# godk1122/IsaacLab

Measured on AMD Instinct MI355X. Metric: env-steps/sec (whole node), Anymal-C rough 4096 envs/GPU, RSL-RL PPO iteration (collect+GAE+update), higher is better.
Workload: dtype f32; 1 GPU; Isaac-Velocity-Rough-Anymal-C-v0, 4096 envs/GPU, T=24, 5 epochs x 4 minibatches, terrain 1204008 triangles, 4 state snapshots resident in HBM; parallelism=dp1, rollout=hipGraph, full_step=False, update=hipGraph (measured eager 16.90 ms, graph 16.30 ms), policy_params=571801

## Files before the change

isaaclab_amd/csrc/mlp.hip:

```cpp
#include <algorithm>

#include "imx_internal.h"

typedef float f32x16 __attribute__((ext_vector_type(16)));

namespace {

constexpr int DW_T = 128;
constexpr int DW_BM = 32;
constexpr int DW_LD = DW_T + 32;

struct DwArgs {
    int64_t M;
    int N, K;
    const float* dY;
    int64_t ldy;
    const float* X;
    int64_t ldx;
    float* part;
    float* part_db;
    int tn, tk, S;
    int64_t rps;
    const float* H;
    int64_t ldh;
// ... 283 lines not shown
    const int64_t i = (int64_t)(blockIdx.x - g.first_block) * 64 + tx;
    const float* src = nullptr;
    int64_t stride = 0;
    float* dst = nullptr;
    if (i < g.total) {
        src = g.part + i; stride = g.total; dst = g.out + i;
    } else if (g.db && i - g.total < g.N) {
        src = g.part_db + (i - g.total); stride = g.N; dst = g.db + (i - g.total);
    }
    float acc = 0.0f;
    if (src)
        for (int s = ty; s < g.S; s += RED_Y) acc += src[(size_t)s * stride];
    red[ty][tx] = acc;
    __syncthreads();
    if (ty == 0 && dst) {
        float sum = 0.0f;
#pragma unroll
        for (int y = 0; y < RED_Y; ++y) sum += red[y][tx];
        *dst = sum;
    }
}

struct DwPlan {
    int tn, tk, S;
    int64_t rps;
};

int g_num_cu = 0;
int g_dw_cu_budget = 0;

DwPlan dw_plan(int64_t M, int N, int K) {
    if (g_num_cu == 0) {
        int dev = 0, cu = 0;
        if (hipGetDevice(&dev) != hipSuccess || hipDeviceGetAttribute(&cu, hipDeviceAttributeMultiprocessorCount, dev) != hipSuccess || cu <= 0)
            cu = 256;
        g_num_cu = cu;
    }
    DwPlan p;
    p.tn = (N + DW_T - 1) / DW_T;
    p.tk = (K + DW_T - 1) / DW_T;
    const int T = p.tn * p.tk;
    const int cus = g_dw_cu_budget > 0 ? std::min(g_dw_cu_budget, g_num_cu) : g_num_cu;
    int64_t S = std::max<int64_t>(1, (int64_t)cus / T);
    S = std::min<int64_t>(S, std::max<int64_t>(1, M / (2 * DW_BM)));
    if (S >= 8) S &= ~(int64_t)7;
    p.rps = ((M + S - 1) / S + DW_BM - 1) / DW_BM * DW_BM;
    p.S = (int)((M + p.rps - 1) / p.rps);
    return p;
}

constexpr int HEAD_A = 64;

#define IMX_HALF_LOG_2PI_F 0.91893853320467274178f
template <bool ELU_IN, int AMAX, int LOSS>
__global__ void __launch_bounds__(256) k_head_fwd(int64_t M, int K, int A, float* __restrict__ h, int64_t ldh,
                                                  const float* __restrict__ W, const float* __restrict__ b, float* __restrict__ y,
                                                  float alpha, imx_head_loss_t L) {
    extern __shared__ float sW[];
    for (int i = threadIdx.x; i < A * K; i += blockDim.x) sW[i] = W[i];
    __syncthreads();
    const int q = threadIdx.x & 3;
    const int64_t row = (int64_t)blockIdx.x * 64 + (threadIdx.x >> 2);
    const bool live = row < M;
    float acc[AMAX];
#pragma unroll
    for (int o = 0; o < AMAX; ++o) acc[o] = 0.0f;
    float* hr = h + (live ? row : 0) * ldh;
    for (int k = 4 * q; k < K; k += 16) {
        float4 hv = *reinterpret_cast<const float4*>(hr + k);
        if (ELU_IN) {
            const float ex = (expf(fminf(hv.x, 0.0f)) - 1.0f) * alpha, ey = (expf(fminf(hv.y, 0.0f)) - 1.0f) * alpha;
            const float ez = (expf(fminf(hv.z, 0.0f)) - 1.0f) * alpha, ew = (expf(fminf(hv.w, 0.0f)) - 1.0f) * alpha;
            hv.x = hv.x > 0.0f ? hv.x : ex; hv.y = hv.y > 0.0f ? hv.y : ey; hv.z = hv.z > 0.0f ? hv.z : ez; hv.w = hv.w > 0.0f ? hv.w : ew;
            if (live) *reinterpret_cast<float4*>(hr + k) = hv;
        }
#pragma unroll
        for (int o = 0; o < AMAX; ++o)
            if (o < A) {
                const float4 wv = *reinterpret_cast<const float4*>(sW + o * K + k);
                acc[o] = fmaf(hv.w, wv.w, fmaf(hv.z, wv.z, fmaf(hv.y, wv.y, fmaf(hv.x, wv.x, acc[o]))));
            }
    }
#pragma unroll
    for (int o = 0; o < AMAX; ++o) {
        float v = acc[o];
        v += __shfl_xor(v, 1);
        v += __shfl_xor(v, 2);
        acc[o] = v + b[o < A ? o : 0];
    }
    if (q == 0 && live) {
#pragma unroll
        for (int o = 0; o < AMAX; ++o)
            if (o < A) y[row * A + o] = acc[o];
        if (LOSS == 1) {
            const float inv_m = L.grad_scale / (float)M;
            float logp = 0.0f;
#pragma unroll
            for (int o = 0; o < AMAX; ++o)
                if (o < A) {
                    const float m = acc[o], s = L.sigma_d[row * L.sigma_stride + o];
                    const float d = L.actions_d[row * A + o] - m;
                    logp += -(d * d) / (2.0f * s * s) - logf(s) - IMX_HALF_LOG_2PI_F;
                }
            const float ratio = expf(logp - L.old_logp_d[row]);
            const float ad = L.advantages_d[row], clip = L.clip_param;
            const float s1 = -ad * ratio, s2 = -ad * fminf(fmaxf(ratio, 1.0f - clip), 1.0f + clip);
            float dsur_dlogp;
            if (s1 >= s2) dsur_dlogp = -ad * ratio;
            else dsur_dlogp = (ratio > 1.0f - clip && ratio < 1.0f + clip) ? -ad * ratio : 0.0f;
            const float g = dsur_dlogp * inv_m;
#pragma unroll
            for (int o = 0; o < AMAX; ++o)
                if (o < A) {
                    const float m = acc[o], s = L.sigma_d[row * L.sigma_stride + o];
                    const float d = L.actions_d[row * A + o] - m;
                    L.dmu_d[row * A + o] = g * (d / (s * s));
                    L.dsigma_d[row * A + o] = g * ((d * d) / (s * s * s) - 1.0f / s) - L.entropy_coef * inv_m / s;
                }
        } else if (LOSS == 2) {
            const float inv_m = L.grad_scale / (float)M;
            const float v = acc[0], R = L.returns_d[row], clip = L.clip_param;
            float dv;
            if (L.use_clipped_value_loss) {
                const float vo = L.old_values_d[row];
                const float dlt = v - vo;
                const float vc = vo + fminf(fmaxf(dlt, -clip), clip);
                const float l1 = (v - R) * (v - R), l2 = (vc - R) * (vc - R);
                if (l1 >= l2) dv = 2.0f * (v - R);
                else dv = (dlt > -clip && dlt < clip) ? 2.0f * (vc - R) : 0.0f;
            } else {
                dv = -2.0f * (R - v);
            }
            L.dvalue_d[row] = L.value_loss_coef * dv * inv_m;
        }
    }
}

template <int AB>
__global__ void __launch_bounds__(512) k_head_bwd(int64_t M, int K, int A, const float* __restrict__ dY, const float* __restrict__ h,
                                                    int64_t ldh, const float* __restrict__ W, float alpha, int has_act,
                                                    float* __restrict__ dprev, float* __restrict__ part, float* __restrict__ part_db) {
    const int lane = threadIdx.x & 63, kb = threadIdx.x >> 6, r = lane & 31, half = lane >> 5;
    const int kc = kb * 32 + r;
    const int steps = (A + 1) >> 1;
    float wreg[AB * 16];
#pragma unroll
    for (int s = 0; s < AB * 16; ++s) {
        const int o = 2 * s + half;
        wreg[s] = (s < steps && o < A) ? W[o * K + kc] : 0.0f;
    }
    f32x16 wacc[AB];
    float dbacc[AB];
#pragma unroll
    for (int b = 0; b < AB; ++b) {
        dbacc[b] = 0.0f;
#pragma unroll
        for (int q = 0; q < 16; ++q) wacc[b][q] = 0.0f;
    }
    __shared__ float sdy[2][32 * (HEAD_A + 1)];
    const int P = A | 1;
    const int64_t nblk = (M + 31) / 32;
    int buf = 0;
    for (int64_t rb = blockIdx.x; rb < nblk; rb += gridDim.x, buf ^= 1) {
        const int64_t m0 = rb * 32;
        {
            const int64_t base = m0 * A, lim = M * (int64_t)A;
            for (int e = threadIdx.x; e < 32 * A; e += blockDim.x) {
                const int row = e / A, col = e - row * A;
                sdy[buf][row * P + col] = base + e < lim ? dY[base + e] : 0.0f;
            }
        }
        __syncthreads();
        const float* __restrict__ ty = sdy[buf];
        float hv[16];
#pragma unroll
        for (int q = 0; q < 16; ++q) {
            const int64_t row = m0 + acc_row(q, half);
            hv[q] = row < M ? h[row * ldh + kc] : 0.0f;
        }
        f32x16 dx;
#pragma unroll
        for (int q = 0; q < 16; ++q) dx[q] = 0.0f;
#pragma unroll
        for (int s = 0; s < AB * 16; ++s)
            if (s < steps) {
                const int o = 2 * s + half;
                const float av = o < A ? ty[r * P + o] : 0.0f;
                dx = __builtin_amdgcn_mfma_f32_32x32x2f32(av, wreg[s], dx, 0, 0, 0);
            }
        if (m0 + 32 <= M) {
#pragma unroll
            for (int q = 0; q < 16; ++q) {
                const float g = (has_act && hv[q] <= 0.0f) ? hv[q] + alpha : 1.0f;
                dprev[(m0 + acc_row(q, half)) * (int64_t)K + kc] = dx[q] * g;
            }
        } else {
#pragma unroll
            for (int q = 0; q < 16; ++q) {
                const int64_t row = m0 + acc_row(q, half);
                const float g = (has_act && hv[q] <= 0.0f) ? hv[q] + alpha : 1.0f;
                if (row < M) dprev[row * (int64_t)K + kc] = dx[q] * g;
            }
        }
#pragma unroll
        for (int q = 0; q < 16; ++q) {
#pragma unroll
            for (int b = 0; b < AB; ++b) {
                const int o = 32 * b + r;
                const float av = o < A ? ty[acc_row(q, half) * P + o] : 0.0f;
                wacc[b] = __builtin_amdgcn_mfma_f32_32x32x2f32(av, hv[q], wacc[b], 0, 0, 0);
                dbacc[b] += av;
            }
        }
    }
    float* p = part + (size_t)blockIdx.x * A * K;
#pragma unroll
    for (int b = 0; b < AB; ++b) {
#pragma unroll
        for (int q = 0; q < 16; ++q) {
            const int o = 32 * b + acc_row(q, half);
            if (o < A) p[o * K + kc] = wacc[b][q];
        }
        if (kb == 0) {
            const float tot = dbacc[b] + __shfl_xor(dbacc[b], 32);
            if (half == 0 && 32 * b + r < A) part_db[(size_t)blockIdx.x * A + 32 * b + r] = tot;
        }
    }
}

template <int K, int AMAX, int LOSS, bool ELU_IN>
__global__ void __launch_bounds__(2 * K) k_head_fused(int64_t M, int A, const float* __restrict__ z, int64_t ldz, const float* __restrict__ W,
                                                      const float* __restrict__ bias, float alpha, float* __restrict__ y, imx_head_loss_t L,
                                                      float* __restrict__ dprev, float* __restrict__ part, float* __restrict__ part_db) {
    constexpr int AB = (AMAX + 31) / 32;
    extern __shared__ float smem[];
    constexpr int P = K + 32;
    const int PA = A | 1;
    float* sW = smem;
    float* sh = sW + ((A * K + 3) & ~3);
    float* sdy = sh + 2 * 32 * P;
    float* sbs = sdy + 32 * PA;
    constexpr int T = 2 * K;
    const int lane = threadIdx.x & 63, kb = threadIdx.x >> 6, r = lane & 31, half = lane >> 5;
    const int kc = kb * 32 + r;
    constexpr int tpr = T >> 5;
    const int frow = threadIdx.x / tpr, fpart = threadIdx.x - frow * tpr;
    for (int i = threadIdx.x; i < A * K; i += T) sW[i] = W[i];
    if (threadIdx.x < AMAX) {
        sbs[threadIdx.x] = threadIdx.x < A ? bias[threadIdx.x] : 0.0f;
        if (LOSS == 1) sbs[AMAX + threadIdx.x] = (threadIdx.x < A && L.sigma_stride == 0) ? L.sigma_d[threadIdx.x] : 1.0f;
    }
    const int steps = (A + 1) >> 1;
    float wreg[AB * 16];
#pragma unroll
    for (int s = 0; s < AB * 16; ++s) {
        const int o = 2 * s + half;
        wreg[s] = (s < steps && o < A) ? W[o * K + kc] : 0.0f;
    }
    f32x16 wacc[AB];
    float dbacc[AB];
#pragma unroll
    for (int b = 0; b < AB; ++b) {
        dbacc[b] = 0.0f;
#pragma unroll
        for (int q = 0; q < 16; ++q) wacc[b][q] = 0.0f;
    }
    constexpr int kq = K >> 2;
    const int64_t nblk = (M + 31) / 32;
    float4 zt[4];
    constexpr int JCAP = LOSS == 1 ? (AMAX + tpr - 1) / tpr : 1;
    float la[JCAP], ls[JCAP], l0 = 0.0f, l1 = 0.0f;
    const bool own_sigma = LOSS == 1 && L.sigma_stride != 0;
    auto load_tile = [&](int64_t rb) {
        {
            const int64_t grow = rb * 32 + frow < M ? rb * 32 + frow : M - 1;
            if (LOSS == 1) {
#pragma unroll
                for (int j = 0; j < JCAP; ++j) {
                    const int o = fpart + tpr * j;
                    la[j] = L.actions_d[grow * A + (o < A ? o : 0)];
// ... 301 lines not shown
    IMX_REQUIRE(t_batch == nullptr, "imx_reduce_batch_begin: another batch is still open on this thread (flush it first)");
    t_batch = b;
    return 0;
}

extern "C" int imx_reduce_batch_flush(imx_reduce_batch_t* b, imx_stream_t stream) {
    IMX_REQUIRE(b && t_batch == b, "imx_reduce_batch_flush: this batch is not the one open on this thread");
    t_batch = nullptr;
    if (b->args.n == 0) return 0;
    hipLaunchKernelGGL(k_mlp_reduce_batch, dim3(b->blocks), dim3(64, RED_Y), 0, (hipStream_t)stream, b->args);
    b->args.n = 0;
    b->blocks = 0;
    IMX_HIP(hipGetLastError());
    return 0;
}

extern "C" int imx_mlp_dw(int64_t M, int N, int K, const float* dY_d, int64_t ldy, const float* X_d, int64_t ldx, float* dW_d,
                          float* db_d, void* scratch_d, size_t scratch_bytes, imx_stream_t stream) {
    return mlp_dw_launch("imx_mlp_dw", M, N, K, dY_d, ldy, nullptr, 0, 0.0f, nullptr, 0, X_d, ldx, dW_d, db_d, scratch_d, scratch_bytes,
                         stream);
}

extern "C" int imx_mlp_dw_elu(int64_t M, int N, int K, const float* dH_d, int64_t ldg, const float* H_d, int64_t ldh, float elu_alpha,
                              float* dZ_out_d, int64_t ldd, const float* X_d, int64_t ldx, float* dW_d, float* db_d, void* scratch_d,
                              size_t scratch_bytes, imx_stream_t stream) {
    IMX_REQUIRE(H_d, "imx_mlp_dw_elu: the saved activation output is required");
    return mlp_dw_launch("imx_mlp_dw_elu", M, N, K, dH_d, ldg, H_d, ldh, elu_alpha, dZ_out_d, ldd, X_d, ldx, dW_d, db_d, scratch_d,
                         scratch_bytes, stream);
}

static int head_fwd_launch(int64_t M, int K, int A, float* h_d, int64_t ldh, const float* W_d, const float* b_d, float* y_d,
                           int elu_in_place, float elu_alpha, const imx_head_loss_t* loss, imx_stream_t stream) {
    IMX_REQUIRE(M > 0 && h_d && W_d && b_d && y_d, "imx_mlp_head_fwd: bad arguments");
    IMX_REQUIRE(A >= 1 && A <= HEAD_A, "imx_mlp_head_fwd: %d outputs (1..%d supported; wider layers are library GEMMs)", A, HEAD_A);
    IMX_REQUIRE(K >= 16 && K % 16 == 0 && K <= 2048 && ldh >= K && ldh % 4 == 0 && aligned16(h_d),
                "imx_mlp_head_fwd: in-features %d (pitch %lld) must be a multiple of 16, 16-byte aligned rows", K, (long long)ldh);
    IMX_REQUIRE((size_t)A * K * sizeof(float) <= 64 * 1024, "imx_mlp_head_fwd: %d x %d weights do not fit the 64 KB of LDS used", A, K);
    imx_head_loss_t L{};
    int mode = 0;
    if (loss) {
        L = *loss;
        mode = L.mode;
        IMX_REQUIRE(mode == 1 || mode == 2, "imx_mlp_head_fwd_loss: mode %d (1 policy, 2 value)", mode);
        if (mode == 1) {
            IMX_REQUIRE(L.sigma_d && L.actions_d && L.old_logp_d && L.advantages_d && L.dmu_d && L.dsigma_d, "imx_mlp_head_fwd_loss: null policy argument");
            IMX_REQUIRE(L.sigma_stride == 0 || L.sigma_stride == A, "imx_mlp_head_fwd_loss: sigma_stride must be 0 (shared std) or A");
        } else {
            IMX_REQUIRE(A == 1 && L.returns_d && L.dvalue_d && (!L.use_clipped_value_loss || L.old_values_d), "imx_mlp_head_fwd_loss: value head needs A = 1, returns, old values");
        }
    }
    const dim3 grid((unsigned)((M + 63) / 64)), block(256);
    const size_t lds = (size_t)A * K * sizeof(float);
    hipStream_t st = (hipStream_t)stream;
#define IMX_HEAD_FWD(E, AM, LS) hipLaunchKernelGGL((k_head_fwd<E, AM, LS>), grid, block, lds, st, M, K, A, h_d, ldh, W_d, b_d, y_d, elu_alpha, L)
#define IMX_HEAD_FWD_E(AM, LS) do { if (elu_in_place) IMX_HEAD_FWD(true, AM, LS); else IMX_HEAD_FWD(false, AM, LS); } while (0)
    if (A <= 16) {
        if (mode == 0) IMX_HEAD_FWD_E(16, 0); else if (mode == 1) IMX_HEAD_FWD_E(16, 1); else IMX_HEAD_FWD_E(16, 2);
    } else {
        if (mode == 0) IMX_HEAD_FWD_E(HEAD_A, 0); else if (mode == 1) IMX_HEAD_FWD_E(HEAD_A, 1); else IMX_HEAD_FWD_E(HEAD_A, 2);
    }
#undef IMX_HEAD_FWD_E
#undef IMX_HEAD_FWD
    IMX_HIP(hipGetLastError());
    return 0;
}

extern "C" int imx_mlp_head_fwd(int64_t M, int K, int A, float* h_d, int64_t ldh, const float* W_d, const float* b_d, float* y_d,
                                int elu_in_place, float elu_alpha, imx_stream_t stream) {
    return head_fwd_launch(M, K, A, h_d, ldh, W_d, b_d, y_d, elu_in_place, elu_alpha, nullptr, stream);
}

extern "C" int imx_mlp_head_fwd_loss(int64_t M, int K, int A, float* h_d, int64_t ldh, const float* W_d, const float* b_d, float* y_d,
                                     int elu_in_place, float elu_alpha, const imx_head_loss_t* loss, imx_stream_t stream) {
    IMX_REQUIRE(loss, "imx_mlp_head_fwd_loss: null loss description");
    return head_fwd_launch(M, K, A, h_d, ldh, W_d, b_d, y_d, elu_in_place, elu_alpha, loss, stream);
}

extern "C" int imx_mlp_head_bwd(int64_t M, int K, int A, const float* dY_d, const float* h_d, int64_t ldh, const float* W_d, float elu_alpha,
                                int has_activation, float* dprev_d, float* dW_d, float* db_d, void* scratch_d, size_t scratch_bytes,
                                imx_stream_t stream) {
    IMX_REQUIRE(M > 0 && dY_d && h_d && W_d && dprev_d && dW_d && db_d && scratch_d, "imx_mlp_head_bwd: bad arguments");
    IMX_REQUIRE(A >= 1 && A <= HEAD_A, "imx_mlp_head_bwd: %d outputs (1..%d supported)", A, HEAD_A);
    IMX_REQUIRE(K >= 32 && K % 32 == 0 && K <= 256 && ldh >= K, "imx_mlp_head_bwd: in-features %d must be a multiple of 32, at most 256", K);
    const int G = head_grid(M);
    const size_t need = ((size_t)G * A * K + (size_t)G * A) * sizeof(float);
    IMX_REQUIRE(scratch_bytes >= need, "imx_mlp_head_bwd: scratch too small (%zu < %zu bytes)", scratch_bytes, need);
    float* part = (float*)scratch_d;
    float* part_db = part + (size_t)G * A * K;
    hipStream_t st = (hipStream_t)stream;
    if (A <= 32)
        hipLaunchKernelGGL((k_head_bwd<1>), dim3((unsigned)G), dim3((unsigned)(K / 32 * 64)), 0, st, M, K, A, dY_d, h_d, ldh, W_d, elu_alpha,
                           has_activation, dprev_d, part, part_db);
    else
        hipLaunchKernelGGL((k_head_bwd<2>), dim3((unsigned)G), dim3((unsigned)(K / 32 * 64)), 0, st, M, K, A, dY_d, h_d, ldh, W_d, elu_alpha,
                           has_activation, dprev_d, part, part_db);
    IMX_HIP(hipGetLastError());
    return reduce_or_defer("imx_mlp_head_bwd", (int64_t)A * K, G, part, dW_d, A, part_db, db_d, st);
}

extern "C" int imx_mlp_head_fwd_bwd(int64_t M, int K, int A, const float* z_d, int64_t ldz, const float* W_d, const float* b_d, float* y_d,
                                    int elu_in, float elu_alpha, const imx_head_loss_t* loss, float* dprev_d, float* dW_d, float* db_d,
                                    void* scratch_d, size_t scratch_bytes, imx_reduce_batch_t* defer_to, imx_stream_t stream) {
    IMX_REQUIRE(M > 0 && z_d && W_d && b_d && y_d && loss && dprev_d && dW_d && db_d && scratch_d, "imx_mlp_head_fwd_bwd: bad arguments");
    IMX_REQUIRE(A >= 1 && A <= HEAD_A, "imx_mlp_head_fwd_bwd: %d outputs (1..%d supported)", A, HEAD_A);
    IMX_REQUIRE((K == 128 || K == 256) && ldz >= K && ldz % 4 == 0 && aligned16(z_d),
                "imx_mlp_head_fwd_bwd: in-features %d (pitch %lld) must be 128 or 256 with 16-byte aligned rows", K, (long long)ldz);
    IMX_REQUIRE(A <= 16, "imx_mlp_head_fwd_bwd: %d outputs (at most 16: wider heads run as imx_mlp_head_fwd_loss + imx_mlp_head_bwd)", A);
    const imx_head_loss_t L = *loss;
    IMX_REQUIRE(L.mode == 1 || L.mode == 2, "imx_mlp_head_fwd_bwd: loss mode %d (1 = policy, 2 = value)", L.mode);
    if (L.mode == 1) {
        IMX_REQUIRE(L.sigma_d && L.actions_d && L.old_logp_d && L.advantages_d && L.dmu_d && L.dsigma_d, "imx_mlp_head_fwd_bwd: null policy argument");
        IMX_REQUIRE(L.sigma_stride == 0 || L.sigma_stride == A, "imx_mlp_head_fwd_bwd: sigma_stride must be 0 (shared std) or A");
    } else {
        IMX_REQUIRE(A == 1 && L.returns_d && L.dvalue_d && (!L.use_clipped_value_loss || L.old_values_d),
                    "imx_mlp_head_fwd_bwd: value head needs A = 1, returns, old values");
    }
    const int G = head_grid(M);
    const size_t need = ((size_t)G * A * K + (size_t)G * A) * sizeof(float);
    IMX_REQUIRE(scratch_bytes >= need, "imx_mlp_head_fwd_bwd: scratch too small (%zu < %zu bytes)", scratch_bytes, need);
    float* part = (float*)scratch_d;
    float* part_db = part + (size_t)G * A * K;
    hipStream_t st = (hipStream_t)stream;
    const size_t lds = ((size_t)((A * K + 3) & ~3) + 2ull * 32 * (K + 32) + 32ull * (A | 1) + 2 * HEAD_A) * sizeof(float);
    const dim3 grid((unsigned)G), block((unsigned)(2 * K));
#define IMX_HEAD_FUSED(K_, AM, LS, E)                                                                                                      \
    do {                                                                                                                                  \
        static bool attr = false;                                                                                                         \
        if (!attr) {                                                                                                                      \
            IMX_HIP(hipFuncSetAttribute(reinterpret_cast<const void*>(k_head_fused<K_, AM, LS, E>), hipFuncAttributeMaxDynamicSharedMemorySize, \
                                        160 * 1024));                                                                                    \
            attr = true;                                                                                                                  \
        }                                                                                                                                 \
        hipLaunchKernelGGL((k_head_fused<K_, AM, LS, E>), grid, block, lds, st, M, A, z_d, ldz, W_d, b_d, elu_alpha, y_d, L, dprev_d, part, \
                           part_db);                                                                                                      \
    } while (0)
#define IMX_HEAD_FUSED_K(AM, LS, E) do { if (K == 128) IMX_HEAD_FUSED(128, AM, LS, E); else IMX_HEAD_FUSED(256, AM, LS, E); } while (0)
    if (L.mode == 2) {
        if (elu_in) IMX_HEAD_FUSED_K(1, 2, true); else IMX_HEAD_FUSED_K(1, 2, false);
    } else {
        if (elu_in) IMX_HEAD_FUSED_K(16, 1, true); else IMX_HEAD_FUSED_K(16, 1, false);
    }
#undef IMX_HEAD_FUSED_K
#undef IMX_HEAD_FUSED
    IMX_HIP(hipGetLastError());
    if (defer_to) {
        imx_reduce_batch* saved = t_batch;
        t_batch = defer_to;
        const int rc = reduce_or_defer("imx_mlp_head_fwd_bwd", (int64_t)A * K, G, part, dW_d, A, part_db, db_d, st);
// ... 535 lines not shown
```

isaaclab_amd/csrc/rollout.hip:

```cpp
#include "imx_internal.h"

struct Mom {
    float n, mean, m2;
};
IMX_DEV Mom mom_merge(Mom a, Mom b) {
    Mom r;
    r.n = a.n + b.n;
    if (r.n == 0.0f) { r.mean = 0.0f; r.m2 = 0.0f; return r; }
    const float d = b.mean - a.mean;
    r.mean = a.mean + d * (b.n / r.n);
    r.m2 = a.m2 + b.m2 + d * d * (a.n * b.n / r.n);
    return r;
}
IMX_DEV Mom mom_wave(Mom m) {
#pragma unroll
    for (int o = 32; o > 0; o >>= 1) {
        Mom b;
        b.n = __shfl_xor(m.n, o, 64);
        b.mean = __shfl_xor(m.mean, o, 64);
        b.m2 = __shfl_xor(m.m2, o, 64);
        const bool lo = ((threadIdx.x & o) == 0);
        m = lo ? mom_merge(m, b) : mom_merge(b, m);
    }
    return m;
// ... 126 lines not shown
    for (int u = GAE_TMAX - 1; u >= 0; --u) {
        if (u < T) {
            const float nnt = 1.0f - (d[u] ? 1.0f : 0.0f);
            const float delta = r[u] + nnt * gamma * next_v - v[u];
            advantage = delta + nnt * gamma * lam * advantage;
            const float rt = advantage + v[u];
            const float at = rt - v[u];
            if (live) {
                ret[(int64_t)u * N + e] = rt;
                adv[(int64_t)u * N + e] = at;
            }
            m.n += 1.0f;
            const float dd = at - m.mean;
            m.mean += dd / m.n;
            m.m2 += dd * (at - m.mean);
            next_v = v[u];
        }
    }
    if (!live) m = Mom{0.0f, 0.0f, 0.0f};
    m = mom_wave(m);
    if (threadIdx.x == 0) {
        scratch[3 * blockIdx.x + 0] = m.n;
        scratch[3 * blockIdx.x + 1] = m.mean;
        scratch[3 * blockIdx.x + 2] = m.m2;
    }
}

extern "C" int imx_gae(int64_t T, int64_t N, const float* rew, const float* val, const uint8_t* dones,
                       const float* last_val, float gamma, float lam, int normalize, float* ret, float* adv,
                       void* scratch, imx_stream_t stream) {
    IMX_REQUIRE(T > 0 && N > 0, "imx_gae: empty rollout (T=%lld N=%lld)", (long long)T, (long long)N);
    IMX_REQUIRE(rew && val && dones && last_val && ret && adv && scratch, "imx_gae: null argument");
    const unsigned nblk = (unsigned)((N + GAE_BLOCK - 1) / GAE_BLOCK);
    if (T <= GAE_TMAX)
        hipLaunchKernelGGL(k_gae_short, dim3(nblk), dim3(GAE_BLOCK), 0, (hipStream_t)stream, (int)T, N, rew, val, dones, last_val, gamma, lam,
                           ret, adv, (float*)scratch);
    else
        hipLaunchKernelGGL(k_gae, dim3(nblk), dim3(GAE_BLOCK), 0, (hipStream_t)stream, T, N, rew, val, dones, last_val, gamma, lam,
                           ret, adv, (float*)scratch);
    IMX_HIP(hipGetLastError());
    if (normalize) {
        const int64_t total = T * N;
        const unsigned grid = (unsigned)std::min<int64_t>((total / 4 + 255) / 256 + 1, 1024);
        hipLaunchKernelGGL(k_adv_normalize, dim3(grid), dim3(256), 0, (hipStream_t)stream, total, (int)nblk,
                           (const float*)scratch, adv);
        IMX_HIP(hipGetLastError());
    }
    return 0;
}


extern "C" size_t imx_ppo_scratch_bytes(int64_t M) { return ((size_t)((M + 255) / 256) * 4 + 8) * sizeof(float); }

__global__ void __launch_bounds__(256)
k_ppo_fwd(int64_t M, int A, const float* __restrict__ mu, const float* __restrict__ sigma, int sigma_stride,
          const float* __restrict__ act, const float* __restrict__ old_logp, const float* __restrict__ old_mu,
          const float* __restrict__ old_sigma, const float* __restrict__ adv, const float* __restrict__ ret,
          const float* __restrict__ val, const float* __restrict__ old_val, float clip, int clipped_value,
          float* __restrict__ part) {
    const int64_t i = (int64_t)blockIdx.x * blockDim.x + threadIdx.x;
    float sur = 0.0f, vl = 0.0f, ent = 0.0f, kl = 0.0f;
    if (i < M) {
        float logp = 0.0f;
        for (int a = 0; a < A; ++a) {
            const float m = mu[i * A + a], s = sigma[i * sigma_stride + a];
            const float d = act[i * A + a] - m;
            const float ls = logf(s);
            logp += -(d * d) / (2.0f * s * s) - ls - IMX_HALF_LOG_2PI;
            ent += 0.5f + IMX_HALF_LOG_2PI + ls;
            if (old_mu) {
                const float mo = old_mu[i * A + a], so = old_sigma[i * A + a];
                const float dm = mo - m;
                kl += logf(s / so + 1.0e-5f) + (so * so + dm * dm) / (2.0f * s * s) - 0.5f;
            }
        }
        const float ratio = expf(logp - old_logp[i]);
        const float ad = adv[i];
        const float s1 = -ad * ratio, s2 = -ad * fminf(fmaxf(ratio, 1.0f - clip), 1.0f + clip);
        sur = fmaxf(s1, s2);
        const float v = val[i], R = ret[i];
        if (clipped_value) {
            const float vo = old_val[i];
            const float vc = vo + fminf(fmaxf(v - vo, -clip), clip);
            const float l1 = (v - R) * (v - R), l2 = (vc - R) * (vc - R);
            vl = fmaxf(l1, l2);
        } else {
            vl = (R - v) * (R - v);
        }
    }
    __shared__ float sm[4][4];
    float r4[4] = {sur, vl, ent, kl};
#pragma unroll
    for (int q = 0; q < 4; ++q) {
        float x = r4[q];
#pragma unroll
        for (int o = 32; o > 0; o >>= 1) x += __shfl_xor(x, o, 64);
        if ((threadIdx.x & 63) == 0) sm[threadIdx.x >> 6][q] = x;
    }
    __syncthreads();
    if (threadIdx.x < 4) part[4 * blockIdx.x + threadIdx.x] = (sm[0][threadIdx.x] + sm[1][threadIdx.x]) + (sm[2][threadIdx.x] + sm[3][threadIdx.x]);
}

__global__ void k_ppo_finish(int nblk, float inv_m, float vcoef, float ecoef, const float* __restrict__ part,
                             float* __restrict__ out8, float* __restrict__ accum) {
    __shared__ float red[16][4];
    __shared__ float r[4];
    const int q = threadIdx.x & 3, chunk = threadIdx.x >> 2;
    float s = 0.0f;
    for (int b = chunk; b < nblk; b += 16) s += part[4 * b + q];
    red[chunk][q] = s;
    __syncthreads();
    if (threadIdx.x < 4) {
        float tot = 0.0f;
        for (int c = 0; c < 16; ++c) tot += red[c][threadIdx.x];
        r[threadIdx.x] = tot * inv_m;
        out8[threadIdx.x] = r[threadIdx.x];
    }
    __syncthreads();
    if (threadIdx.x == 0) {
        out8[4] = r[0] + vcoef * r[1] - ecoef * r[2];
        if (accum) {
            accum[0] += r[1]; accum[1] += r[0]; accum[2] += r[2]; accum[3] += r[3]; accum[4] += 1.0f;
        }
    }
}

// ... 4 lines not shown
          int clipped_value, float vcoef, float ecoef, float gscale, float* __restrict__ dmu,
          float* __restrict__ dsigma, float* __restrict__ dval) {
    const int64_t i = (int64_t)blockIdx.x * blockDim.x + threadIdx.x;
    if (i >= M) return;
    const float inv_m = gscale / (float)M;
    if (dmu) {
        float logp = 0.0f;
        for (int a = 0; a < A; ++a) {
            const float m = mu[i * A + a], s = sigma[i * sigma_stride + a];
            const float d = act[i * A + a] - m;
            logp += -(d * d) / (2.0f * s * s) - logf(s) - IMX_HALF_LOG_2PI;
        }
        const float ratio = expf(logp - old_logp[i]);
        const float ad = adv[i];
        const float s1 = -ad * ratio, s2 = -ad * fminf(fmaxf(ratio, 1.0f - clip), 1.0f + clip);
        float dsur_dlogp;
        if (s1 >= s2) dsur_dlogp = -ad * ratio;
        else dsur_dlogp = (ratio > 1.0f - clip && ratio < 1.0f + clip) ? -ad * ratio : 0.0f;
        const float g = dsur_dlogp * inv_m;
        for (int a = 0; a < A; ++a) {
            const float m = mu[i * A + a], s = sigma[i * sigma_stride + a];
            const float d = act[i * A + a] - m;
            dmu[i * A + a] = g * (d / (s * s));
            dsigma[i * A + a] = g * ((d * d) / (s * s * s) - 1.0f / s) - ecoef * inv_m / s;
        }
    }
    if (!dval) return;
    const float v = val[i], R = ret[i];
    float dv;
    if (clipped_value) {
        const float vo = old_val[i];
        const float dlt = v - vo;
        const float vc = vo + fminf(fmaxf(dlt, -clip), clip);
        const float l1 = (v - R) * (v - R), l2 = (vc - R) * (vc - R);
        if (l1 >= l2) dv = 2.0f * (v - R);
        else dv = (dlt > -clip && dlt < clip) ? 2.0f * (vc - R) : 0.0f;
    } else {
        dv = -2.0f * (R - v);
    }
    dval[i] = vcoef * dv * inv_m;
}

extern "C" int imx_ppo_loss_fwd(int64_t M, int64_t A, const float* mu, const float* sigma, int64_t sigma_stride,
                                const float* act, const float* old_logp, const float* old_mu, const float* old_sigma,
                                const float* adv, const float* ret, const float* val, const float* old_val, float clip,
                                int clipped_value, float vcoef, float ecoef, float* out8, float* accum, void* scratch,
                                imx_stream_t stream) {
    IMX_REQUIRE(M > 0 && A > 0 && A <= 4096, "imx_ppo_loss_fwd: bad sizes M=%lld A=%lld", (long long)M, (long long)A);
    IMX_REQUIRE(sigma_stride == 0 || sigma_stride == A, "imx_ppo_loss_fwd: sigma_stride must be 0 (shared std) or A");
    IMX_REQUIRE(mu && sigma && act && old_logp && adv && ret && val && out8 && scratch, "imx_ppo_loss_fwd: null argument");
    IMX_REQUIRE(!clipped_value || old_val, "imx_ppo_loss_fwd: clipped value loss needs old values");
    IMX_REQUIRE((old_mu == nullptr) == (old_sigma == nullptr), "imx_ppo_loss_fwd: old_mu/old_sigma must come together");
    const unsigned nblk = (unsigned)((M + 255) / 256);
    hipLaunchKernelGGL(k_ppo_fwd, dim3(nblk), dim3(256), 0, (hipStream_t)stream, M, (int)A, mu, sigma, (int)sigma_stride, act,
                       old_logp, old_mu, old_sigma, adv, ret, val, old_val, clip, clipped_value, (float*)scratch);
    hipLaunchKernelGGL(k_ppo_finish, dim3(1), dim3(64), 0, (hipStream_t)stream, (int)nblk, 1.0f / (float)M, vcoef, ecoef,
                       (const float*)scratch, out8, accum);
    IMX_HIP(hipGetLastError());
    return 0;
}

extern "C" int imx_ppo_loss_bwd(int64_t M, int64_t A, const float* mu, const float* sigma, int64_t sigma_stride,
                                const float* act, const float* old_logp, const float* adv, const float* ret, const float* val,
                                const float* old_val, float clip, int clipped_value, float vcoef, float ecoef, float gscale,
                                float* dmu, float* dsigma, float* dval, imx_stream_t stream) {
    IMX_REQUIRE(M > 0 && A > 0, "imx_ppo_loss_bwd: bad sizes");
    IMX_REQUIRE(sigma_stride == 0 || sigma_stride == A, "imx_ppo_loss_bwd: sigma_stride must be 0 (shared std) or A");
    IMX_REQUIRE(dmu || dval, "imx_ppo_loss_bwd: nothing to compute (dmu and dval are both null)");
    IMX_REQUIRE(!dmu || (mu && sigma && act && old_logp && adv && dsigma), "imx_ppo_loss_bwd: the policy part needs mu, sigma, "
                "actions, old log-prob, advantages and dsigma");
    IMX_REQUIRE(!dval || (ret && val), "imx_ppo_loss_bwd: the value part needs returns and values");
    IMX_REQUIRE(!dval || !clipped_value || old_val, "imx_ppo_loss_bwd: clipped value loss needs old values");
    hipLaunchKernelGGL(k_ppo_bwd, dim3((unsigned)((M + 255) / 256)), dim3(256), 0, (hipStream_t)stream, M, (int)A, mu, sigma,
                       (int)sigma_stride, act, old_logp, adv, ret, val, old_val, clip, clipped_value, vcoef, ecoef, gscale, dmu,
                       dsigma, dval);
    IMX_HIP(hipGetLastError());
    return 0;
}

__global__ void __launch_bounds__(256)
k_adam(int64_t n, float* __restrict__ p, const float* __restrict__ g, float* __restrict__ m, float* __restrict__ v,
       const float* __restrict__ lr_d, const float* __restrict__ norm_d, float max_norm, float b1, float b2, float eps,
       float bias1, float sqrt_bias2) {
    const float lr = lr_d[0];
    float coef = 1.0f;
    if (norm_d) coef = fminf(max_norm / (norm_d[0] + 1.0e-6f), 1.0f);
    const float step_size = lr / bias1;
    for (int64_t i = (int64_t)blockIdx.x * blockDim.x + threadIdx.x; i < n; i += (int64_t)gridDim.x * blockDim.x) {
        const float gi = g[i] * coef;
        const float mi = b1 * m[i] + (1.0f - b1) * gi;
        const float vi = b2 * v[i] + (1.0f - b2) * gi * gi;
        m[i] = mi;
        v[i] = vi;
        p[i] = p[i] - step_size * (mi / (sqrtf(vi) / sqrt_bias2 + eps));
    }
}

extern "C" int imx_adam_step(int64_t n, float* p, const float* g, float* m, float* v, const float* lr_d,
                             const float* grad_norm_d, float max_norm, float beta1, float beta2, float eps,
                             int64_t step, imx_stream_t stream) {
    IMX_REQUIRE(n > 0 && p && g && m && v && lr_d && step > 0, "imx_adam_step: bad arguments");
    const float bias1 = 1.0f - powf(beta1, (float)step);
    const float sb2 = sqrtf(1.0f - powf(beta2, (float)step));
    const unsigned grid = (unsigned)std::min<int64_t>((n + 255) / 256, 2048);
    hipLaunchKernelGGL(k_adam, dim3(grid), dim3(256), 0, (hipStream_t)stream, n, p, g, m, v, lr_d, grad_norm_d, max_norm,
                       beta1, beta2, eps, bias1, sb2);
    IMX_HIP(hipGetLastError());
    return 0;
// ... 316 lines not shown
```

Baseline: 5.238 million env-steps/s.

## Specialize MLP head kernels for K=128/256 with prefetch and software pipelining

Adds compile-time K specializations to the head forward kernel. Activations and loss inputs are loaded before the weight copy into shared memory, so global latency overlaps the weight staging. Adds a software-pipelined head backward kernel that fetches the next row block of dY and h into registers while MFMA work runs on the current block. Also specializes the PPO loss forward for A=12/37, batching all loads ahead of the math. The cost is more register pressure and more template instances, and the specialized paths only cover the listed sizes.

```diff
diff --git a/isaaclab_amd/csrc/mlp.hip b/isaaclab_amd/csrc/mlp.hip
--- a/isaaclab_amd/csrc/mlp.hip
+++ b/isaaclab_amd/csrc/mlp.hip
@@ -359,13 +359,44 @@
 constexpr int HEAD_A = 64;
 
 #define IMX_HALF_LOG_2PI_F 0.91893853320467274178f
-template <bool ELU_IN, int AMAX, int LOSS>
+__device__ __forceinline__ float4 head_elu4(float4 hv, float alpha) {
+    const float ex = (expf(fminf(hv.x, 0.0f)) - 1.0f) * alpha, ey = (expf(fminf(hv.y, 0.0f)) - 1.0f) * alpha;
+    const float ez = (expf(fminf(hv.z, 0.0f)) - 1.0f) * alpha, ew = (expf(fminf(hv.w, 0.0f)) - 1.0f) * alpha;
+    hv.x = hv.x > 0.0f ? hv.x : ex; hv.y = hv.y > 0.0f ? hv.y : ey; hv.z = hv.z > 0.0f ? hv.z : ez; hv.w = hv.w > 0.0f ? hv.w : ew;
+    return hv;
+}
+
+template <int AMAX>
+__device__ __forceinline__ void head_dot4(float (&acc)[AMAX], float4 hv, const float* sWk, int K, int A) {
+#pragma unroll
+    for (int o = 0; o < AMAX; ++o)
+        if (o < A) {
+            const float4 wv = *reinterpret_cast<const float4*>(sWk + o * K);
+            acc[o] = fmaf(hv.w, wv.w, fmaf(hv.z, wv.z, fmaf(hv.y, wv.y, fmaf(hv.x, wv.x, acc[o]))));
+        }
+}
+
+template <int NMAX>
+__device__ __forceinline__ void head_weights_to_lds(float* sW, const float* __restrict__ W, int n) {
+#pragma unroll
+    for (int c = 0; c < (NMAX + 2047) / 2048; ++c) {
+        const int i0 = c * 2048 + threadIdx.x;
+        if (c * 2048 < n) {
+            float w[8];
+#pragma unroll
+            for (int j = 0; j < 8; ++j) w[j] = W[min(i0 + 256 * j, n - 1)];
+#pragma unroll
+            for (int j = 0; j < 8; ++j)
+                if (i0 + 256 * j < n) sW[i0 + 256 * j] = w[j];
+        }
+    }
+}
+
+template <bool ELU_IN, int AMAX, int LOSS, int KT>
 __global__ void __launch_bounds__(256) k_head_fwd(int64_t M, int K, int A, float* __restrict__ h, int64_t ldh,
                                                   const float* __restrict__ W, const float* __restrict__ b, float* __restrict__ y,
                                                   float alpha, imx_head_loss_t L) {
     extern __shared__ float sW[];
-    for (int i = threadIdx.x; i < A * K; i += blockDim.x) sW[i] = W[i];
-    __syncthreads();
     const int q = threadIdx.x & 3;
     const int64_t row = (int64_t)blockIdx.x * 64 + (threadIdx.x >> 2);
     const bool live = row < M;
@@ -373,20 +404,53 @@
 #pragma unroll
     for (int o = 0; o < AMAX; ++o) acc[o] = 0.0f;
     float* hr = h + (live ? row : 0) * ldh;
-    for (int k = 4 * q; k < K; k += 16) {
-        float4 hv = *reinterpret_cast<const float4*>(hr + k);
+    constexpr bool PRE = LOSS != 0 && AMAX <= 16;
+    float pa[PRE && LOSS == 1 ? AMAX : 1], ps[PRE && LOSS == 1 ? AMAX : 1], p0 = 0.0f, p1 = 0.0f;
+    if constexpr (PRE) {
+        const int64_t rc = live ? row : 0;
+        if (LOSS == 1) {
+#pragma unroll
+            for (int o = 0; o < AMAX; ++o) {
+                pa[o] = L.actions_d[rc * A + (o < A ? o : 0)];
+                ps[o] = L.sigma_d[rc * L.sigma_stride + (o < A ? o : 0)];
+            }
+            p0 = L.old_logp_d[rc];
+            p1 = L.advantages_d[rc];
+        } else {
+            p0 = L.returns_d[rc];
+            p1 = L.use_clipped_value_loss ? L.old_values_d[rc] : 0.0f;
+        }
+    }
+    auto sig = [&](int o) { if constexpr (PRE) return ps[o]; else return L.sigma_d[row * L.sigma_stride + o]; };
+    auto act = [&](int o) { if constexpr (PRE) return pa[o]; else return L.actions_d[row * A + o]; };
+    if constexpr (KT > 0) {
+        constexpr int NT = KT / 16;
+        float4 hv[NT];
+#pragma unroll
+        for (int t = 0; t < NT; ++t) hv[t] = *reinterpret_cast<const float4*>(hr + 4 * q + 16 * t);
+        head_weights_to_lds<AMAX * KT>(sW, W, A * KT);
+        __syncthreads();
         if (ELU_IN) {
-            const float ex = (expf(fminf(hv.x, 0.0f)) - 1.0f) * alpha, ey = (expf(fminf(hv.y, 0.0f)) - 1.0f) * alpha;
-            const float ez = (expf(fminf(hv.z, 0.0f)) - 1.0f) * alpha, ew = (expf(fminf(hv.w, 0.0f)) - 1.0f) * alpha;
-            hv.x = hv.x > 0.0f ? hv.x : ex; hv.y = hv.y > 0.0f ? hv.y : ey; hv.z = hv.z > 0.0f ? hv.z : ez; hv.w = hv.w > 0.0f ? hv.w : ew;
-            if (live) *reinterpret_cast<float4*>(hr + k) = hv;
-        }
-#pragma unroll
-        for (int o = 0; o < AMAX; ++o)
-            if (o < A) {
-                const float4 wv = *reinterpret_cast<const float4*>(sW + o * K + k);
-                acc[o] = fmaf(hv.w, wv.w, fmaf(hv.z, wv.z, fmaf(hv.y, wv.y, fmaf(hv.x, wv.x, acc[o]))));
-            }
+#pragma unroll
+            for (int t = 0; t < NT; ++t) hv[t] = head_elu4(hv[t], alpha);
+            if (live) {
+#pragma unroll
+                for (int t = 0; t < NT; ++t) *reinterpret_cast<float4*>(hr + 4 * q + 16 * t) = hv[t];
+            }
+        }
+#pragma unroll
+        for (int t = 0; t < NT; ++t) head_dot4<AMAX>(acc, hv[t], sW + 4 * q + 16 * t, KT, A);
+    } else {
+        for (int i = threadIdx.x; i < A * K; i += 256) sW[i] = W[i];
+        __syncthreads();
+        for (int k = 4 * q; k < K; k += 16) {
+            float4 hv = *reinterpret_cast<const float4*>(hr + k);
+            if (ELU_IN) {
+                hv = head_elu4(hv, alpha);
+                if (live) *reinterpret_cast<float4*>(hr + k) = hv;
+            }
+            head_dot4<AMAX>(acc, hv, sW + k, K, A);
+        }
     }
 #pragma unroll
     for (int o = 0; o < AMAX; ++o) {
@@ -405,12 +469,12 @@
 #pragma unroll
             for (int o = 0; o < AMAX; ++o)
                 if (o < A) {
-                    const float m = acc[o], s = L.sigma_d[row * L.sigma_stride + o];
-                    const float d = L.actions_d[row * A + o] - m;
+                    const float m = acc[o], s = sig(o);
+                    const float d = act(o) - m;
                     logp += -(d * d) / (2.0f * s * s) - logf(s) - IMX_HALF_LOG_2PI_F;
                 }
-            const float ratio = expf(logp - L.old_logp_d[row]);
-            const float ad = L.advantages_d[row], clip = L.clip_param;
+            const float ratio = expf(logp - (PRE ? p0 : L.old_logp_d[row]));
+            const float ad = PRE ? p1 : L.advantages_d[row], clip = L.clip_param;
             const float s1 = -ad * ratio, s2 = -ad * fminf(fmaxf(ratio, 1.0f - clip), 1.0f + clip);
             float dsur_dlogp;
             if (s1 >= s2) dsur_dlogp = -ad * ratio;
@@ -419,17 +483,17 @@
 #pragma unroll
             for (int o = 0; o < AMAX; ++o)
                 if (o < A) {
-                    const float m = acc[o], s = L.sigma_d[row * L.sigma_stride + o];
-                    const float d = L.actions_d[row * A + o] - m;
+                    const float m = acc[o], s = sig(o);
+                    const float d = act(o) - m;
                     L.dmu_d[row * A + o] = g * (d / (s * s));
                     L.dsigma_d[row * A + o] = g * ((d * d) / (s * s * s) - 1.0f / s) - L.entropy_coef * inv_m / s;
                 }
         } else if (LOSS == 2) {
             const float inv_m = L.grad_scale / (float)M;
-            const float v = acc[0], R = L.returns_d[row], clip = L.clip_param;
+            const float v = acc[0], R = PRE ? p0 : L.returns_d[row], clip = L.clip_param;
             float dv;
             if (L.use_clipped_value_loss) {
-                const float vo = L.old_values_d[row];
+                const float vo = PRE ? p1 : L.old_values_d[row];
                 const float dlt = v - vo;
                 const float vc = vo + fminf(fmaxf(dlt, -clip), clip);
                 const float l1 = (v - R) * (v - R), l2 = (vc - R) * (vc - R);
@@ -439,6 +503,69 @@
                 dv = -2.0f * (R - v);
             }
             L.dvalue_d[row] = L.value_loss_coef * dv * inv_m;
+        }
+    }
+}
+
+template <int AB>
+__device__ __forceinline__ void head_bwd_block(int64_t M, int K, int A, int64_t m0, const float* __restrict__ ty, const float (&hv)[16],
+                                               const float (&wreg)[AB * 16], float alpha, int has_act, float* __restrict__ dprev,
+                                               f32x16 (&wacc)[AB], float (&dbacc)[AB]) {
+    const int lane = threadIdx.x & 63, kb = threadIdx.x >> 6, r = lane & 31, half = lane >> 5;
+    const int kc = kb * 32 + r;
+    const int steps = (A + 1) >> 1, P = A | 1;
+    f32x16 dx;
+#pragma unroll
+    for (int q = 0; q < 16; ++q) dx[q] = 0.0f;
+#pragma unroll
+    for (int s = 0; s < AB * 16; ++s)
+        if (s < steps) {
+            const int o = 2 * s + half;
+            const float av = o < A ? ty[r * P + o] : 0.0f;
+            dx = __builtin_amdgcn_mfma_f32_32x32x2f32(av, wreg[s], dx, 0, 0, 0);
+        }
+    if (m0 + 32 <= M) {
+#pragma unroll
+        for (int q = 0; q < 16; ++q) {
+            const float g = (has_act && hv[q] <= 0.0f) ? hv[q] + alpha : 1.0f;
+            dprev[(m0 + acc_row(q, half)) * (int64_t)K + kc] = dx[q] * g;
+        }
+    } else {
+#pragma unroll
+        for (int q = 0; q < 16; ++q) {
+            const int64_t row = m0 + acc_row(q, half);
+            const float g = (has_act && hv[q] <= 0.0f) ? hv[q] + alpha : 1.0f;
+            if (row < M) dprev[row * (int64_t)K + kc] = dx[q] * g;
+        }
+    }
+#pragma unroll
+    for (int q = 0; q < 16; ++q) {
+#pragma unroll
+        for (int b = 0; b < AB; ++b) {
+            const int o = 32 * b + r;
+            const float av = o < A ? ty[acc_row(q, half) * P + o] : 0.0f;
+            wacc[b] = __builtin_amdgcn_mfma_f32_32x32x2f32(av, hv[q], wacc[b], 0, 0, 0);
+            dbacc[b] += av;
+        }
+    }
+}
+
+template <int AB>
+__device__ __forceinline__ void head_bwd_partials(int K, int A, const f32x16 (&wacc)[AB], const float (&dbacc)[AB], float* __restrict__ part,
+                                                  float* __restrict__ part_db) {
+    const int lane = threadIdx.x & 63, kb = threadIdx.x >> 6, r = lane & 31, half = lane >> 5;
+    const int kc = kb * 32 + r;
+    float* p = part + (size_t)blockIdx.x * A * K;
+#pragma unroll
+    for (int b = 0; b < AB; ++b) {
+#pragma unroll
+        for (int q = 0; q < 16; ++q) {
+            const int o = 32 * b + acc_row(q, half);
+            if (o < A) p[o * K + kc] = wacc[b][q];
+        }
+        if (kb == 0) {
+            const float tot = dbacc[b] + __shfl_xor(dbacc[b], 32);
+            if (half == 0 && 32 * b + r < A) part_db[(size_t)blockIdx.x * A + 32 * b + r] = tot;
         }
     }
 }
@@ -478,61 +605,82 @@
             }
         }
         __syncthreads();
-        const float* __restrict__ ty = sdy[buf];
         float hv[16];
 #pragma unroll
         for (int q = 0; q < 16; ++q) {
             const int64_t row = m0 + acc_row(q, half);
             hv[q] = row < M ? h[row * ldh + kc] : 0.0f;
         }
-        f32x16 dx;
-#pragma unroll
-        for (int q = 0; q < 16; ++q) dx[q] = 0.0f;
-#pragma unroll
-        for (int s = 0; s < AB * 16; ++s)
-            if (s < steps) {
-                const int o = 2 * s + half;
-                const float av = o < A ? ty[r * P + o] : 0.0f;
-                dx = __builtin_amdgcn_mfma_f32_32x32x2f32(av, wreg[s], dx, 0, 0, 0);
-            }
-        if (m0 + 32 <= M) {
-#pragma unroll
-            for (int q = 0; q < 16; ++q) {
-                const float g = (has_act && hv[q] <= 0.0f) ? hv[q] + alpha : 1.0f;
-                dprev[(m0 + acc_row(q, half)) * (int64_t)K + kc] = dx[q] * g;
-            }
-        } else {
-#pragma unroll
-            for (int q = 0; q < 16; ++q) {
-                const int64_t row = m0 + acc_row(q, half);
-                const float g = (has_act && hv[q] <= 0.0f) ? hv[q] + alpha : 1.0f;
-                if (row < M) dprev[row * (int64_t)K + kc] = dx[q] * g;
-            }
+        head_bwd_block<AB>(M, K, A, m0, sdy[buf], hv, wreg, alpha, has_act, dprev, wacc, dbacc);
+    }
+    head_bwd_partials<AB>(K, A, wacc, dbacc, part, part_db);
+}
+
+template <int AB, int KT>
+__global__ void __launch_bounds__(2 * KT) k_head_bwd_pipe(int64_t M, int A, const float* __restrict__ dY, const float* __restrict__ h,
+                                                          int64_t ldh, const float* __restrict__ W, float alpha, int has_act,
+                                                          float* __restrict__ dprev, float* __restrict__ part, float* __restrict__ part_db) {
+    constexpr int K = KT, T = 2 * KT;
+    constexpr int DYR = (32 * 32 * AB + T - 1) / T;
+    const int lane = threadIdx.x & 63, kb = threadIdx.x >> 6, r = lane & 31, half = lane >> 5;
+    const int kc = kb * 32 + r;
+    const int steps = (A + 1) >> 1;
+    float wreg[AB * 16];
+#pragma unroll
+    for (int s = 0; s < AB * 16; ++s) {
+        const int o = 2 * s + half;
+        wreg[s] = (s < steps && o < A) ? W[o * K + kc] : 0.0f;
+    }
+    f32x16 wacc[AB];
+    float dbacc[AB];
+#pragma unroll
+    for (int b = 0; b < AB; ++b) {
+        dbacc[b] = 0.0f;
+#pragma unroll
+        for (int q = 0; q < 16; ++q) wacc[b][q] = 0.0f;
+    }
+    __shared__ float sdy[2][32 * (HEAD_A + 1)];
+    const int P = A | 1;
+    const int64_t nblk = (M + 31) / 32, lim = M * (int64_t)A;
+    int soff[DYR];
+#pragma unroll
+    for (int j = 0; j < DYR; ++j) {
+        const int e = threadIdx.x + T * j, row = e / A;
+        soff[j] = e < 32 * A ? row * P + (e - row * A) : -1;
+    }
+    float hn[16], dyn[DYR];
+    auto request = [&](int64_t rb) {
+        const int64_t m0 = rb * 32, base = m0 * A;
+#pragma unroll
+        for (int j = 0; j < DYR; ++j) {
+            const int64_t e = base + threadIdx.x + T * j;
+            dyn[j] = dY[e < lim ? e : lim - 1];
         }
 #pragma unroll
         for (int q = 0; q < 16; ++q) {
-#pragma unroll
-            for (int b = 0; b < AB; ++b) {
-                const int o = 32 * b + r;
-                const float av = o < A ? ty[acc_row(q, half) * P + o] : 0.0f;
-                wacc[b] = __builtin_amdgcn_mfma_f32_32x32x2f32(av, hv[q], wacc[b], 0, 0, 0);
-                dbacc[b] += av;
-            }
-        }
-    }
-    float* p = part + (size_t)blockIdx.x * A * K;
-#pragma unroll
-    for (int b = 0; b < AB; ++b) {
-#pragma unroll
-        for (int q = 0; q < 16; ++q) {
-            const int o = 32 * b + acc_row(q, half);
-            if (o < A) p[o * K + kc] = wacc[b][q];
-        }
-        if (kb == 0) {
-            const float tot = dbacc[b] + __shfl_xor(dbacc[b], 32);
-            if (half == 0 && 32 * b + r < A) part_db[(size_t)blockIdx.x * A + 32 * b + r] = tot;
-        }
-    }
+            const int64_t row = m0 + acc_row(q, half);
+            hn[q] = h[(row < M ? row : M - 1) * ldh + kc];
+        }
+    };
+    auto stage = [&](float* slab, int64_t rb) {
+#pragma unroll
+        for (int j = 0; j < DYR; ++j)
+            if (soff[j] >= 0) slab[soff[j]] = rb * 32 * A + threadIdx.x + T * j < lim ? dyn[j] : 0.0f;
+    };
+    request(blockIdx.x);
+    stage(sdy[0], blockIdx.x);
+    int buf = 0;
+    for (int64_t rb = blockIdx.x; rb < nblk; rb += gridDim.x, buf ^= 1) {
+        float hv[16];
+#pragma unroll
+        for (int q = 0; q < 16; ++q) hv[q] = rb * 32 + acc_row(q, half) < M ? hn[q] : 0.0f;
+        __syncthreads();
+        const bool more = rb + gridDim.x < nblk;
+        if (more) request(rb + gridDim.x);
+        head_bwd_block<AB>(M, K, A, rb * 32, sdy[buf], hv, wreg, alpha, has_act, dprev, wacc, dbacc);
+        if (more) stage(sdy[buf ^ 1], rb + gridDim.x);
+    }
+    head_bwd_partials<AB>(K, A, wacc, dbacc, part, part_db);
 }
 
 template <int K, int AMAX, int LOSS, bool ELU_IN>
@@ -940,7 +1088,8 @@
     const dim3 grid((unsigned)((M + 63) / 64)), block(256);
     const size_t lds = (size_t)A * K * sizeof(float);
     hipStream_t st = (hipStream_t)stream;
-#define IMX_HEAD_FWD(E, AM, LS) hipLaunchKernelGGL((k_head_fwd<E, AM, LS>), grid, block, lds, st, M, K, A, h_d, ldh, W_d, b_d, y_d, elu_alpha, L)
+#define IMX_HEAD_FWD_K(E, AM, LS, KT) hipLaunchKernelGGL((k_head_fwd<E, AM, LS, KT>), grid, block, lds, st, M, K, A, h_d, ldh, W_d, b_d, y_d, elu_alpha, L)
+#define IMX_HEAD_FWD(E, AM, LS) do { if (K == 128) IMX_HEAD_FWD_K(E, AM, LS, 128); else if (K == 256) IMX_HEAD_FWD_K(E, AM, LS, 256); else IMX_HEAD_FWD_K(E, AM, LS, 0); } while (0)
 #define IMX_HEAD_FWD_E(AM, LS) do { if (elu_in_place) IMX_HEAD_FWD(true, AM, LS); else IMX_HEAD_FWD(false, AM, LS); } while (0)
     if (A <= 16) {
         if (mode == 0) IMX_HEAD_FWD_E(16, 0); else if (mode == 1) IMX_HEAD_FWD_E(16, 1); else IMX_HEAD_FWD_E(16, 2);
@@ -949,6 +1098,7 @@
     }
 #undef IMX_HEAD_FWD_E
 #undef IMX_HEAD_FWD
+#undef IMX_HEAD_FWD_K
     IMX_HIP(hipGetLastError());
     return 0;
 }
@@ -976,12 +1126,19 @@
     float* part = (float*)scratch_d;
     float* part_db = part + (size_t)G * A * K;
     hipStream_t st = (hipStream_t)stream;
-    if (A <= 32)
+#define IMX_HEAD_BWD_PIPE(AB_, KT) hipLaunchKernelGGL((k_head_bwd_pipe<AB_, KT>), dim3((unsigned)G), dim3(2 * KT), 0, st, M, A, dY_d, h_d, ldh, \
+                                                      W_d, elu_alpha, has_activation, dprev_d, part, part_db)
+    if (K == 128 && A <= 32) IMX_HEAD_BWD_PIPE(1, 128);
+    else if (K == 128) IMX_HEAD_BWD_PIPE(2, 128);
+    else if (K == 256 && A <= 32) IMX_HEAD_BWD_PIPE(1, 256);
+    else if (K == 256) IMX_HEAD_BWD_PIPE(2, 256);
+    else if (A <= 32)
         hipLaunchKernelGGL((k_head_bwd<1>), dim3((unsigned)G), dim3((unsigned)(K / 32 * 64)), 0, st, M, K, A, dY_d, h_d, ldh, W_d, elu_alpha,
                            has_activation, dprev_d, part, part_db);
     else
         hipLaunchKernelGGL((k_head_bwd<2>), dim3((unsigned)G), dim3((unsigned)(K / 32 * 64)), 0, st, M, K, A, dY_d, h_d, ldh, W_d, elu_alpha,
                            has_activation, dprev_d, part, part_db);
+#undef IMX_HEAD_BWD_PIPE
     IMX_HIP(hipGetLastError());
     return reduce_or_defer("imx_mlp_head_bwd", (int64_t)A * K, G, part, dW_d, A, part_db, db_d, st);
 }
diff --git a/isaaclab_amd/csrc/rollout.hip b/isaaclab_amd/csrc/rollout.hip
--- a/isaaclab_amd/csrc/rollout.hip
+++ b/isaaclab_amd/csrc/rollout.hip
@@ -202,6 +202,18 @@
 
 extern "C" size_t imx_ppo_scratch_bytes(int64_t M) { return ((size_t)((M + 255) / 256) * 4 + 8) * sizeof(float); }
 
+__device__ __forceinline__ void ppo_fwd_term(float m, float s, float a, float& logp, float& ent) {
+    const float d = a - m;
+    const float ls = logf(s);
+    logp += -(d * d) / (2.0f * s * s) - ls - IMX_HALF_LOG_2PI;
+    ent += 0.5f + IMX_HALF_LOG_2PI + ls;
+}
+__device__ __forceinline__ void ppo_fwd_kl_term(float m, float s, float mo, float so, float& kl) {
+    const float dm = mo - m;
+    kl += logf(s / so + 1.0e-5f) + (so * so + dm * dm) / (2.0f * s * s) - 0.5f;
+}
+
+template <int AT>
 __global__ void __launch_bounds__(256)
 k_ppo_fwd(int64_t M, int A, const float* __restrict__ mu, const float* __restrict__ sigma, int sigma_stride,
           const float* __restrict__ act, const float* __restrict__ old_logp, const float* __restrict__ old_mu,
@@ -212,16 +224,27 @@
     float sur = 0.0f, vl = 0.0f, ent = 0.0f, kl = 0.0f;
     if (i < M) {
         float logp = 0.0f;
-        for (int a = 0; a < A; ++a) {
-            const float m = mu[i * A + a], s = sigma[i * sigma_stride + a];
-            const float d = act[i * A + a] - m;
-            const float ls = logf(s);
-            logp += -(d * d) / (2.0f * s * s) - ls - IMX_HALF_LOG_2PI;
-            ent += 0.5f + IMX_HALF_LOG_2PI + ls;
-            if (old_mu) {
-                const float mo = old_mu[i * A + a], so = old_sigma[i * A + a];
-                const float dm = mo - m;
-                kl += logf(s / so + 1.0e-5f) + (so * so + dm * dm) / (2.0f * s * s) - 0.5f;
+        if constexpr (AT > 0) {
+            float m[AT], s[AT], a_[AT], mo[AT], so[AT];
+#pragma unroll
+            for (int a = 0; a < AT; ++a) {
+                m[a] = mu[i * AT + a];
+                s[a] = sigma[i * sigma_stride + a];
+                a_[a] = act[i * AT + a];
+                mo[a] = old_mu[i * AT + a];
+                so[a] = old_sigma[i * AT + a];
+            }
+            __builtin_amdgcn_sched_barrier(0);
+#pragma unroll
+            for (int a = 0; a < AT; ++a) {
+                ppo_fwd_term(m[a], s[a], a_[a], logp, ent);
+                ppo_fwd_kl_term(m[a], s[a], mo[a], so[a], kl);
+            }
+        } else {
+            for (int a = 0; a < A; ++a) {
+                const float m = mu[i * A + a], s = sigma[i * sigma_stride + a];
+                ppo_fwd_term(m, s, act[i * A + a], logp, ent);
+                if (old_mu) ppo_fwd_kl_term(m, s, old_mu[i * A + a], old_sigma[i * A + a], kl);
             }
         }
         const float ratio = expf(logp - old_logp[i]);
@@ -332,8 +355,13 @@
     IMX_REQUIRE(!clipped_value || old_val, "imx_ppo_loss_fwd: clipped value loss needs old values");
     IMX_REQUIRE((old_mu == nullptr) == (old_sigma == nullptr), "imx_ppo_loss_fwd: old_mu/old_sigma must come together");
     const unsigned nblk = (unsigned)((M + 255) / 256);
-    hipLaunchKernelGGL(k_ppo_fwd, dim3(nblk), dim3(256), 0, (hipStream_t)stream, M, (int)A, mu, sigma, (int)sigma_stride, act,
-                       old_logp, old_mu, old_sigma, adv, ret, val, old_val, clip, clipped_value, (float*)scratch);
+#define IMX_PPO_FWD(AT) hipLaunchKernelGGL((k_ppo_fwd<AT>), dim3(nblk), dim3(256), 0, (hipStream_t)stream, M, (int)A, mu, sigma, \
+                                                (int)sigma_stride, act, old_logp, old_mu, old_sigma, adv, ret, val, old_val, clip, clipped_value, \
+                                                (float*)scratch)
+    if (A == 12 && old_mu) IMX_PPO_FWD(12);
+    else if (A == 37 && old_mu) IMX_PPO_FWD(37);
+    else IMX_PPO_FWD(0);
+#undef IMX_PPO_FWD
     hipLaunchKernelGGL(k_ppo_finish, dim3(1), dim3(64), 0, (hipStream_t)stream, (int)nblk, 1.0f / (float)M, vcoef, ecoef,
                        (const float*)scratch, out8, accum);
     IMX_HIP(hipGetLastError());
```

New measurement: 5.134 million env-steps/s (median of 2 runs). -2.0%, worse.
